# KoryakovDmitry/cuda-mpi-openmp

Hardware: AMD Instinct MI355X
Metric: Gpixel/s lab2 2D conv 4096x4096 + GPU/CPU speedup, at 1/2/4/8 MI355X (higher is better)
Workload: dtype fp32

## Files before the change

### native/src/kernels/edge_kernels.hpp

```cpp
#pragma once

#include <type_traits>

#include "internal.hpp"
#include "peer_sync.hpp"

namespace mpx {
namespace edge {

struct Taps {
    float wx[MPX_MAX_K * MPX_MAX_K];
    float wy[MPX_MAX_K * MPX_MAX_K];
};

struct RowSrc {
    const uint32_t *up = nullptr;
    const uint32_t *dn = nullptr;
    int own_rows = 0x7fffffff;
};

constexpr float kSqrtMargin = 1.0f / 16384.0f;

template <bool FAST>
__device__ __forceinline__ uint32_t mag_to_gray(float s) {
    if constexpr (!FAST) {
        return mpx_sat_u8(sqrtf(s));
    } else {
        if (s >= 65025.0f) return 255u;
        const float r = __builtin_amdgcn_sqrtf(s);
        const float n = truncf(r);
        const float fr = r - n;
        if (fr > kSqrtMargin && fr < 1.0f - kSqrtMargin) return (uint32_t)n;
        return mpx_sat_u8(sqrtf(s));
    }
}

__device__ __forceinline__ void mag2_to_gray(float s0, float s1, uint32_t &g0, uint32_t &g1) {
    const float c0 = __builtin_amdgcn_fmed3f(s0, 0.25f, 65280.25f);
    const float c1 = __builtin_amdgcn_fmed3f(s1, 0.25f, 65280.25f);
    const float r0 = __builtin_amdgcn_sqrtf(c0), r1 = __builtin_amdgcn_sqrtf(c1);
    const float f0 = __builtin_amdgcn_fractf(r0), f1 = __builtin_amdgcn_fractf(r1);
    constexpr float kHalfOpen = 0.5f - kSqrtMargin;
    const bool ok = (int)(fabsf(f0 - 0.5f) < kHalfOpen) & (int)(fabsf(f1 - 0.5f) < kHalfOpen);
    g0 = (uint32_t)r0;
    g1 = (uint32_t)r1;
    if (!ok) {
        g0 = mpx_sat_u8(sqrtf(s0));
        g1 = mpx_sat_u8(sqrtf(s1));
    }
}

typedef float f2_t __attribute__((ext_vector_type(2)));

__device__ __forceinline__ void mag4_to_gray(f2_t s01, f2_t s23, uint32_t g[4]) {
    constexpr float kTwo23 = 8388608.0f;
    const f2_t c01 = {__builtin_amdgcn_fmed3f(s01.x, 0.25f, 65280.25f), __builtin_amdgcn_fmed3f(s01.y, 0.25f, 65280.25f)};
    const f2_t c23 = {__builtin_amdgcn_fmed3f(s23.x, 0.25f, 65280.25f), __builtin_amdgcn_fmed3f(s23.y, 0.25f, 65280.25f)};
    const f2_t r01 = {__builtin_amdgcn_sqrtf(c01.x), __builtin_amdgcn_sqrtf(c01.y)};
    const f2_t r23 = {__builtin_amdgcn_sqrtf(c23.x), __builtin_amdgcn_sqrtf(c23.y)};
    const f2_t kp = {-0.5f + kSqrtMargin, -0.5f + kSqrtMargin}, km = {-0.5f - kSqrtMargin, -0.5f - kSqrtMargin};
    const f2_t big = {kTwo23, kTwo23};
    const f2_t p01 = (r01 + kp) + big, m01 = (r01 + km) + big;
    const f2_t p23 = (r23 + kp) + big, m23 = (r23 + km) + big;
    const bool ok = (int)(p01.x == m01.x) & (int)(p01.y == m01.y) & (int)(p23.x == m23.x) & (int)(p23.y == m23.y);
    if (ok) {
        typedef uint32_t u2_t __attribute__((ext_vector_type(2)));
        const u2_t b01 = __builtin_bit_cast(u2_t, p01), b23 = __builtin_bit_cast(u2_t, p23);
        g[0] = b01.x;
        g[1] = b01.y;
        g[2] = b23.x;
        g[3] = b23.y;
    } else {
        g[0] = mpx_sat_u8(sqrtf(s01.x));
        g[1] = mpx_sat_u8(sqrtf(s01.y));
        g[2] = mpx_sat_u8(sqrtf(s23.x));
        g[3] = mpx_sat_u8(sqrtf(s23.y));
    }
}

template <int MODE, bool FAST>
__device__ __forceinline__ uint32_t finish_gray(float gx, float gy) {
    if constexpr (MODE == MPX_CONV_MAG2) {
        const float a = gx * gx;
        const float b = gy * gy;
        return mag_to_gray<FAST>(a + b);
    } else if constexpr (MODE == MPX_CONV_ABS1) {
        return mpx_sat_u8(fabsf(gx));
    } else {
        return mpx_sat_u8(gx);
    }
}

constexpr int kTX = 64;
constexpr int kTY = 4;
constexpr int kCPT = 2;
constexpr int kTW = kTX * kCPT;
constexpr int kHL = 4;
constexpr int kLW = kTW + 2 * kHL;
constexpr int kNVROW = kLW / 4;

template <bool VEC>
__device__ __forceinline__ uint4 fetch4(const uint32_t *__restrict__ row, int gx, int w) {
    if constexpr (VEC) {
        const int gxc = mpx_clampi(gx, 0, w - 4);
        const uint4 q = *reinterpret_cast<const uint4 *>(row + gxc);
        const bool left = gx < 0, right = gx >= w;
        uint4 p;
        p.x = right ? q.w : q.x;
        p.y = left ? q.x : (right ? q.w : q.y);
        p.z = left ? q.x : (right ? q.w : q.z);
        p.w = left ? q.x : q.w;
        return p;
    } else {
        uint4 p;
        p.x = row[mpx_clampi(gx + 0, 0, w - 1)];
        p.y = row[mpx_clampi(gx + 1, 0, w - 1)];
        p.z = row[mpx_clampi(gx + 2, 0, w - 1)];
        p.w = row[mpx_clampi(gx + 3, 0, w - 1)];
        return p;
    }
}

__device__ __forceinline__ float4 luma4(uint4 p) {
    return make_float4(mpx_luma(p.x), mpx_luma(p.y), mpx_luma(p.z), mpx_luma(p.w));
}

__device__ __forceinline__ uint32_t alpha4(uint4 p) {
    return (p.x >> 24) | ((p.y >> 24) << 8) | ((p.z >> 24) << 16) | (p.w & 0xff000000u);
}

template <int K, int A, int MODE, int RPT, bool FAST>
__device__ __forceinline__ void tile_compute(const float *__restrict__ lum, const Taps &taps, int tx, int ty,
                                             uint32_t (&res)[RPT][kCPT]) {
    constexpr int OFF = (kHL - A) & 1;
    constexpr int NW = (OFF + kCPT + K - 1 + 1) / 2;
    constexpr bool TWO = (MODE == MPX_CONV_MAG2);
    const int wbase = kCPT * tx + kHL - A - OFF;
    float ax[RPT][kCPT], ay[RPT][kCPT];
#pragma unroll
    for (int o = 0; o < RPT; ++o)
#pragma unroll
        for (int j = 0; j < kCPT; ++j) {
            ax[o][j] = 0.0f;
            ay[o][j] = 0.0f;
        }
#pragma unroll
    for (int r = 0; r < RPT + K - 1; ++r) {
        const float *lrow = lum + (ty * RPT + r) * kLW + wbase;
        float wnd[2 * NW];
#pragma unroll
        for (int q = 0; q < NW; ++q) {
            const float2 t = *reinterpret_cast<const float2 *>(lrow + 2 * q);
            wnd[2 * q] = t.x;
            wnd[2 * q + 1] = t.y;
        }
#pragma unroll
        for (int o = 0; o < RPT; ++o) {
            const int dy = r - o;
            if (dy < 0 || dy >= K) continue;
#pragma unroll
            for (int dx = 0; dx < K; ++dx) {
                const float cx = taps.wx[dy * K + dx];
#pragma unroll
                for (int j = 0; j < kCPT; ++j) ax[o][j] = fmaf(cx, wnd[OFF + j + dx], ax[o][j]);
                if constexpr (TWO) {
                    const float cy = taps.wy[dy * K + dx];
#pragma unroll
                    for (int j = 0; j < kCPT; ++j) ay[o][j] = fmaf(cy, wnd[OFF + j + dx], ay[o][j]);
                }
            }
        }
    }
#pragma unroll
    for (int o = 0; o < RPT; ++o)
#pragma unroll
        for (int j = 0; j < kCPT; ++j) res[o][j] = finish_gray<MODE, FAST>(ax[o][j], ay[o][j]);
}

template <int K, int A, int MODE, int RPT, bool VEC, bool FAST>
__global__ __launch_bounds__(256) void conv_stream_kernel(const uint32_t *__restrict__ in, uint32_t *__restrict__ out,
                                                          int w, int pitch, int oy0, int oy1, int y_lo, int y_hi,
                                                          int tiles_y, int chunk, int chunks_per_strip, Taps taps) {
    constexpr int TH = kTY * RPT;
    constexpr int LH = TH + K - 1;
    constexpr int HALO = K - 1;
    constexpr int NEWV = TH * kNVROW;
    constexpr int ITN = (NEWV + 255) / 256;
    constexpr int LUMF = LH * kLW;
    static_assert(A <= kHL && (K - 1 - A) <= kHL, "window exceeds loaded halo");
    static_assert(TH >= HALO, "tile shorter than the window");
    __shared__ __attribute__((aligned(16))) float smem[LUMF + LH * kTW / 4];
    float *lum = smem;
    uint8_t *alpha = reinterpret_cast<uint8_t *>(smem + LUMF);

    const int tid = threadIdx.x;
    const int tx = tid & (kTX - 1);
    const int ty = __builtin_amdgcn_readfirstlane(tid >> 6);
    const int b = xcd_remap(blockIdx.x, gridDim.x);
    const int strip = b / chunks_per_strip;
    const int t0 = (b - strip * chunks_per_strip) * chunk;
    const int t1 = min(t0 + chunk, tiles_y);
    if (t0 >= t1) return;
    const int x0 = strip * kTW;
    const bool full_x = (x0 + kTW <= w);

    auto fetch_rows = [&](uint4 (&regs)[ITN], int gy_first, int nrows_total) {
// ... 319 lines not shown
            r = *reinterpret_cast<const uint2 *>(row + cc);
        } else if constexpr (VEC) {
            const __amdgpu_buffer_rsrc_t rrow = __builtin_amdgcn_make_buffer_rsrc(const_cast<uint32_t *>(row), 0,
                                                                                  w * 4, 0x00020000);
            typedef uint32_t u32x2_t __attribute__((ext_vector_type(2)));
            const u32x2_t v = __builtin_amdgcn_raw_buffer_load_b64(rrow, i <= i_last ? cc * 4 : 0x7ffffff0, 0, 0);
            r = make_uint2(v.x, v.y);
        } else {
            r = make_uint2(row[mpx_clampi(cin, 0, w - 1)], row[mpx_clampi(cin + 1, 0, w - 1)]);
        }
        __builtin_amdgcn_sched_barrier(0);
        return r;
    };
    auto fix_pair = [&](uint2 q) -> uint2 {
        if constexpr (VEC) {
            uint2 p;
            p.x = pair_right ? q.y : q.x;
            p.y = pair_left ? q.x : q.y;
            return p;
        } else {
            return q;
        }
    };

    constexpr int D = K * ((PF + K - 1) / K);
    uint2 pre[D];
    f2_t we[K][NE];
    f2_t wo[K][NO > 0 ? NO : 1];
    f2_t hxr[K], hyr[K];
    uint32_t alp0[K], alp1[K];

    auto consume = [&](int u, uint2 px) {
        const f2_t l = luma2(px.x, px.y);
        alp0[u] = px.x;
        alp1[u] = px.y;
        float wv[NV];
        wv[A] = l.x;
        wv[A + 1] = l.y;
        if constexpr (A >= 1) wv[A - 1] = from_prev(l.y);
        if constexpr (A >= 2) wv[A - 2] = from_prev(l.x);
        if constexpr (A >= 3) wv[A - 3] = from_prev(wv[A - 1]);
        if constexpr (G::R >= 1) wv[A + 2] = from_next(l.x);
        if constexpr (G::R >= 2) wv[A + 3] = from_next(l.y);
        if constexpr (G::R >= 3) wv[A + 4] = from_next(wv[A + 2]);
        if constexpr (SEP) {
            auto pair = [&](int dx) { return f2_t{wv[dx], wv[dx + 1]}; };
            hxr[u] = sep_chain<F, K, 0>(taps, pair);
            if constexpr (TWO) hyr[u] = sep_chain<F, K, 2>(taps, pair);
        } else {
#pragma unroll
            for (int q = 0; q < NE; ++q) we[u][q] = f2_t{wv[2 * q], 2 * q + 1 < NV ? wv[2 * q + 1] : 0.0f};
#pragma unroll
            for (int q = 0; q < NO; ++q) wo[u][q] = f2_t{wv[2 * q + 1], wv[2 * q + 2]};
        }
    };

#pragma unroll
    for (int q = 0; q < D; ++q) pre[q] = load_row(q);
#pragma unroll
    for (int u = 0; u < K - 1; ++u) {
        const uint2 px = fix_pair(pre[u]);
        pre[u] = load_row(u + D);
        consume(u, px);
    }
    auto row_step = [&](auto upc, int g, int v) {
        constexpr bool UP = decltype(upc)::value;
        const int u = (K - 1 + v) % K;
        const int q = (K - 1 + v) % D;
        const int i = K - 1 + g * D + v;
        const uint2 px = fix_pair(pre[q]);
        pre[q] = load_row(i + D);
        consume(u, px);
        const int y = UP ? ye - 1 - (g * D + v) : ys + g * D + v;
        auto slot = [&](int dy) { return UP ? (u + K - dy) % K : (u + 1 + dy) % K; };
        f2_t gx = {0.0f, 0.0f}, gy = {0.0f, 0.0f};
        if constexpr (SEP) {
            gx = sep_chain<F, K, 1>(taps, [&](int dy) { return hxr[slot(dy)]; });
            const float sx = sep_scale<F, K, false>(taps);
            gx = gx * f2_t{sx, sx};
            if constexpr (TWO) {
                gy = sep_chain<F, K, 3>(taps, [&](int dy) { return hyr[slot(dy)]; });
                const float sy = sep_scale<F, K, true>(taps);
                gy = gy * f2_t{sy, sy};
            }
        } else {
            bool sx = false, sy = false;
#pragma unroll
            for (int dy = 0; dy < K; ++dy) {
                const int r = slot(dy);
#pragma unroll
                for (int dx = 0; dx < K; ++dx) {
                    const f2_t pv = (dx & 1) ? wo[r][dx >> 1] : we[r][dx >> 1];
                    tap_step<F::kConst>(gx, sx, tap_x<F>(taps, dy * K + dx), pv);
                    if constexpr (TWO) tap_step<F::kConst>(gy, sy, tap_y<F>(taps, dy * K + dx), pv);
                }
            }
        }
        uint32_t g0, g1;
        if constexpr (TWO) {
            const f2_t sq = gx * gx + gy * gy;
            if constexpr (FAST) {
                mag2_to_gray(sq.x, sq.y, g0, g1);
            } else {
                g0 = mag_to_gray<false>(sq.x);
                g1 = mag_to_gray<false>(sq.y);
            }
        } else {
            g0 = finish_gray<MODE, FAST>(gx.x, 0.0f);
            g1 = finish_gray<MODE, FAST>(gx.y, 0.0f);
        }
        const uint32_t v0 = __builtin_amdgcn_perm(alp0[slot(A)], g0, 0x07000000u);
        const uint32_t v1 = __builtin_amdgcn_perm(alp1[slot(A)], g1, 0x07000000u);
        const bool row_ok = UP ? y >= ys : y < ye;
        const int yc = row_ok ? y : ys;
        const __amdgpu_buffer_rsrc_t orow =
            __builtin_amdgcn_make_buffer_rsrc(out + (int64_t)yc * pitch, 0, row_ok ? w * 4 : 0, 0x00020000);
        constexpr int kDrop = 0x7ffffff0;
        if constexpr (VEC) {
            typedef uint32_t u32x2_t __attribute__((ext_vector_type(2)));
            const u32x2_t pv = {v0, v1};
            __builtin_amdgcn_raw_buffer_store_b64(pv, orow, st0 ? ox * 4 : kDrop, 0, BUFLD == 3 ? 2 : 0);
        } else {
            __builtin_amdgcn_raw_buffer_store_b32(v0, orow, st0 ? ox * 4 : kDrop, 0, 0);
            __builtin_amdgcn_raw_buffer_store_b32(v1, orow, st1 ? ox * 4 + 4 : kDrop, 0, 0);
        }
    };
    const int nrows = ye - ys;
    const int nfull = nrows / D;
    const int rem = nrows - nfull * D;
    auto run = [&](auto upc) {
        for (int g = 0; g < nfull; ++g) {
#pragma unroll
            for (int v = 0; v < D; ++v) row_step(upc, g, v);
        }
        if (rem > 0) {
#pragma unroll
            for (int v = 0; v < D; ++v) {
                if (v >= rem) break;
                row_step(upc, nfull, v);
            }
        }
    };
    if (up) run(std::true_type{});
    else run(std::false_type{});
}

constexpr int kVsRowWords = 64 * 4 + 4;
constexpr int kVsSlotWords = 2 * kVsRowWords;
struct VsX {
    int take_start = -1, give_start = -1, take_end = -1, give_end = -1;
    int ftake_start = 0, fgive_start = 0, ftake_end = 0, fgive_end = 0;
};

template <int K, int A, int MODE, bool FAST, class F, bool UP, int OPT, bool SPW = false, int VSEG = 0>
__device__ __forceinline__ void band4_walk(const uint32_t *__restrict__ in, uint32_t *__restrict__ out,
                                                     int w, int pitch, int ys, int ye, int y_lo, int y_hi, int x0,
                                                     const Taps &taps, RowSrc rs, uint32_t *mbf = nullptr,
                                                     uint32_t *mbl = nullptr, int nf = 0, int nl = 0,
                                                     uint32_t *lds = nullptr, VsX vx = VsX{}) {
    constexpr int R = K - 1 - A;
    constexpr int NV = 4 + A + R;
    constexpr bool TWO = (MODE == MPX_CONV_MAG2);
    constexpr bool SEP = F::kSep;
    typedef uint32_t u32x4_t __attribute__((ext_vector_type(4)));
    typedef uint32_t u32x2_t __attribute__((ext_vector_type(2)));
    const int lane = threadIdx.x & 63;
    constexpr bool up = UP;
    constexpr bool HL = (OPT & 512) != 0;
    const int cin = HL ? x0 - 4 + 4 * lane : x0 + 4 * lane;
    const bool st = HL ? (lane >= 1 && lane <= 62 && cin < w) : cin < w;
    const int cc = HL ? min(max(cin, 0), w - 4) : min(cin, w - 4);
    const bool q_right = cin >= w;
    const bool q_left = HL && cin < 0;
    const bool ap_left = lane == 0, ap_right = lane == 63;
    const bool ap_have = !HL && !(OPT & 16) && ((ap_left && x0 > 0) || (ap_right && x0 + 256 < w));
    constexpr int kDrop = 0x7ffffff0;
    constexpr bool kDppApron = (OPT & (8 | 16 | 512)) == 0;
    constexpr bool BPA = kDppApron && (OPT & 2048) != 0 && !SPW;
    const bool fix_l = kDppApron && ap_left && x0 == 0, fix_r = kDppApron && ap_right && x0 + 256 >= w;
    const int ap_off = ap_have ? (ap_left ? x0 - 2 : x0 + 256) * 4 : (fix_l ? 0 : (fix_r ? cc * 4 + 8 : kDrop));
    const uint32_t ap_selx = fix_r ? 0x07060504u : 0x03020100u;
    const uint32_t ap_sely = fix_l ? 0x03020100u : 0x07060504u;
    if constexpr (VSEG > 0) ye = ys + VSEG;
    const int iy0 = ys - A;
    const int iy_last = ye - 1 + R;
    auto row_ptr = [&](int i) {
        const int gy = mpx_clampi(up ? iy_last - i : iy0 + i, y_lo, y_hi);
        const uint32_t *src = gy < 0 ? rs.up : (gy >= rs.own_rows ? rs.dn : in);
        return src + (int64_t)gy * pitch;
    };
    const int i_last = ye - ys + K - 2;
    static_assert(VSEG == 0 || (A == 2 && K == 5 && VSEG >= 8), "vertical sharing: 5-row windows, 2 + 2 halo rows");
    auto load_row = [&](int i, u32x2_t &ap) -> u32x4_t {
        const uint32_t *row = row_ptr(min(i, i_last));
        int nrec = scalar_le_sel(i, i_last, w * 4);
        if constexpr (VSEG > 0)
            nrec = ((i < 2 && vx.take_start >= 0) || (i >= VSEG + 2 && vx.take_end >= 0)) ? 0 : nrec;
        const __amdgpu_buffer_rsrc_t rr =
            __builtin_amdgcn_make_buffer_rsrc(const_cast<uint32_t *>(row), 0, nrec, 0x00020000);
        const int qo = cc * 4, ao = ap_off;
        u32x4_t q;
        if constexpr (SPW) {
            q = __builtin_amdgcn_raw_buffer_load_b128(rr, qo, 0, peer::kCpolSystem);
            ap = __builtin_amdgcn_raw_buffer_load_b64(rr, ao, 0, peer::kCpolSystem);
        } else if constexpr (HL) {
            q = __builtin_amdgcn_raw_buffer_load_b128(rr, qo, 0, 0);
            ap = u32x2_t{0u, 0u};
        } else if constexpr ((OPT & 8) != 0) {
            q = __builtin_amdgcn_raw_buffer_load_b128(rr, qo, 0, (OPT & 64) ? 2 : 0);
        } else if constexpr (BPA) {
            if ((OPT & 32) && i >= K - 1 && i < ye - ys)
                q = __builtin_amdgcn_raw_buffer_load_b128(rr, qo, 0, 2);
            else
                q = __builtin_amdgcn_raw_buffer_load_b128(rr, qo, 0, 0);
            ap = u32x2_t{0u, 0u};
        } else if ((OPT & 64) || ((OPT & 32) && i >= K - 1 && i < ye - ys)) {
            q = __builtin_amdgcn_raw_buffer_load_b128(rr, qo, 0, 2);
            ap = __builtin_amdgcn_raw_buffer_load_b64(rr, ao, 0, (OPT & 128) ? 0 : 2);
        } else {
            q = __builtin_amdgcn_raw_buffer_load_b128(rr, qo, 0, 0);
            ap = __builtin_amdgcn_raw_buffer_load_b64(rr, ao, 0, 0);
        }
        __builtin_amdgcn_sched_barrier(0);
        return q;
    };
    auto fix_quad = [&](u32x4_t q) -> u32x4_t {
        if constexpr ((OPT & 1024) != 0) return q;
        if constexpr (HL) {
            if (q_left) return u32x4_t{q.x, q.x, q.x, q.x};
        }
        return q_right ? u32x4_t{q.w, q.w, q.w, q.w} : q;
    };
    f2_t ab = {0.0f, 0.0f};
    int bp_addr = 0;
    if constexpr (BPA) {
        const int nload = ye - ys + K - 1;
        const int j = lane >> 1;
        const bool side = lane & 1;
        const bool edge = side ? x0 + 256 >= w : x0 == 0;
        const int col = side ? (edge ? w - 2 : x0 + 256) : (edge ? 0 : x0 - 2);
        const u32x2_t v = *reinterpret_cast<const u32x2_t *>(row_ptr(min(j, nload - 1)) + col);
        ab = luma2((edge && side) ? v.y : v.x, (edge && !side) ? v.x : v.y);
        bp_addr = ap_right ? 4 : 0;
    }
    if constexpr ((OPT & 8) != 0) {
        const int nload = ye - ys + K - 1;
        const int j = lane >> 1, side = lane & 1;
        const bool have = !(OPT & 16) && (side ? x0 + 256 < w : x0 > 0);
        const uint32_t *row = row_ptr(min(j, nload - 1));
        const u32x2_t v = *reinterpret_cast<const u32x2_t *>(row + (have ? (side ? x0 + 256 : x0 - 2) : 0));
        ab = luma2(v.x, v.y);
    }

    constexpr int D = K * ((4 + K - 1) / K);
    u32x4_t pre[D];
    u32x2_t apr[D];
    f2_t hxr[SEP ? K : 1][2], hyr[SEP ? K : 1][2];
    float win[SEP ? 1 : K][NV];
    uint32_t alp[K], alq[K];

    auto consume = [&](int u, u32x4_t px, u32x2_t ap, int ri) {
        const f2_t l01 = luma2(px.x, px.y), l23 = luma2(px.z, px.w);
        alp[u] = __builtin_amdgcn_perm(px.y, px.x, 0x0c0c0703u);
        alq[u] = __builtin_amdgcn_perm(px.w, px.z, 0x0c0c0703u);
        f2_t la;
        if constexpr ((OPT & 8) != 0) {
            auto rl = [&](float x, int l) {
                return __int_as_float(__builtin_amdgcn_readlane(__float_as_int(x), l));
            };
            const f2_t lft = {rl(ab.x, 2 * ri), rl(ab.y, 2 * ri)};
            const f2_t rgt = {rl(ab.x, 2 * ri + 1), rl(ab.y, 2 * ri + 1)};
            la = ap_left ? lft : rgt;
        } else if constexpr (BPA) {
            const int a = bp_addr + 8 * ri;
            la = f2_t{__int_as_float(__builtin_amdgcn_ds_bpermute(a, __float_as_int(ab.x))),
                      __int_as_float(__builtin_amdgcn_ds_bpermute(a, __float_as_int(ab.y)))};
        } else if constexpr (kDppApron) {
            la = luma2(__builtin_amdgcn_perm(ap.y, ap.x, ap_selx), __builtin_amdgcn_perm(ap.y, ap.x, ap_sely));
        } else {
            la = luma2(ap.x, ap.y);
        }
        float wv[NV];
        wv[A + 0] = l01.x;
        wv[A + 1] = l01.y;
        wv[A + 2] = l23.x;
        wv[A + 3] = l23.y;
        if constexpr (kDppApron) {
            if constexpr (A >= 1) wv[A - 1] = shift_or_old<kDppShr1>(la.y, l23.y);
            if constexpr (A >= 2) wv[A - 2] = shift_or_old<kDppShr1>(la.x, l23.x);
            if constexpr (R >= 1) wv[A + 4] = shift_or_old<kDppShl1>(la.x, l01.x);
            if constexpr (R >= 2) wv[A + 5] = shift_or_old<kDppShl1>(la.y, l01.y);
        } else {
            if constexpr (A >= 1) {
                const float d = from_prev(l23.y);
                wv[A - 1] = ap_left ? (ap_have ? la.y : l01.x) : d;
            }
            if constexpr (A >= 2) {
                const float d = from_prev(l23.x);
                wv[A - 2] = ap_left ? (ap_have ? la.x : l01.x) : d;
            }
            if constexpr (R >= 1) {
                const float d = from_next(l01.x);
                wv[A + 4] = ap_right ? (ap_have ? la.x : l23.y) : d;
            }
            if constexpr (R >= 2) {
                const float d = from_next(l01.y);
                wv[A + 5] = ap_right ? (ap_have ? la.y : l23.y) : d;
            }
        }
        if constexpr (SEP && kDppApron && A == 2 && R == 2) {
            const f2_t e0 = {wv[0], wv[1]}, e3 = {wv[6], wv[7]};
            const f2_t pw[7] = {e0, __builtin_shufflevector(e0, l01, 1, 2), l01, __builtin_shufflevector(l01, l23, 1, 2),
                                l23, __builtin_shufflevector(l23, e3, 1, 2), e3};
#pragma unroll
            for (int e = 0; e < 2; ++e) {
                auto pair = [&](int dx) { return pw[2 * e + dx]; };
                hxr[u][e] = sep_chain<F, K, 0>(taps, pair);
                if constexpr (TWO) hyr[u][e] = sep_chain<F, K, 2>(taps, pair);
            }
        } else if constexpr (SEP) {
#pragma unroll
            for (int e = 0; e < 2; ++e) {
                auto pair = [&](int dx) { return f2_t{wv[2 * e + dx], wv[2 * e + dx + 1]}; };
                hxr[u][e] = sep_chain<F, K, 0>(taps, pair);
                if constexpr (TWO) hyr[u][e] = sep_chain<F, K, 2>(taps, pair);
            }
        } else {
#pragma unroll
            for (int j = 0; j < NV; ++j) win[u][j] = wv[j];
        }
    };

    auto vs_put = [&](int slot, int r, u32x4_t q, u32x2_t ap) {
        *reinterpret_cast<u32x4_t *>(lds + slot + r * kVsRowWords + 4 * lane) = q;
        if (ap_left || ap_right)
            *reinterpret_cast<u32x2_t *>(lds + slot + r * kVsRowWords + 256 + (ap_right ? 2 : 0)) = ap;
    };
    auto vs_get = [&](int slot, int r, u32x2_t &ap) -> u32x4_t {
        if (ap_left || ap_right)
            ap = *reinterpret_cast<const u32x2_t *>(lds + slot + r * kVsRowWords + 256 + (ap_right ? 2 : 0));
        return *reinterpret_cast<const u32x4_t *>(lds + slot + r * kVsRowWords + 4 * lane);
    };
    auto vs_flag = [&](int f) { __hip_atomic_store(lds + f, 1u, __ATOMIC_RELEASE, __HIP_MEMORY_SCOPE_WORKGROUP); };
    auto vs_wait = [&](int f) {
        while (__hip_atomic_load(lds + f, __ATOMIC_ACQUIRE, __HIP_MEMORY_SCOPE_WORKGROUP) == 0u)
            __builtin_amdgcn_s_sleep(1);
    };

#pragma unroll
    for (int q = 0; q < D; ++q) pre[q] = load_row(q, apr[q]);
    if constexpr (VSEG > 0) {
        if (vx.give_start >= 0) {
            vs_put(vx.give_start, UP ? 1 : 0, pre[2], apr[2]);
            vs_put(vx.give_start, UP ? 0 : 1, pre[3], apr[3]);
            vs_flag(vx.fgive_start);
        }
        if (vx.take_start >= 0) {
            vs_wait(vx.ftake_start);
            pre[0] = vs_get(vx.take_start, UP ? 1 : 0, apr[0]);
            pre[1] = vs_get(vx.take_start, UP ? 0 : 1, apr[1]);
        }
    }
#pragma unroll
    for (int u = 0; u < K - 1; ++u) {
        const u32x4_t px = fix_quad(pre[u]);
        const u32x2_t ap = apr[u];
        pre[u] = load_row(u + D, apr[u]);
        consume(u, px, ap, u);
    }
    auto row_step = [&](int g, int v) {
        const int u = (K - 1 + v) % K;
        const int q = (K - 1 + v) % D;
        const int i = K - 1 + g * D + v;
        if constexpr (VSEG > 0) {
            if (vx.give_end >= 0 && (i == VSEG || i == VSEG + 1)) {
                vs_put(vx.give_end, UP ? (i == VSEG ? 1 : 0) : (i == VSEG ? 0 : 1), pre[q], apr[q]);
                if (i == VSEG + 1) vs_flag(vx.fgive_end);
            }
            if (vx.take_end >= 0 && (i == VSEG + 2 || i == VSEG + 3)) {
                if (i == VSEG + 2) vs_wait(vx.ftake_end);
                pre[q] = vs_get(vx.take_end, UP ? (i == VSEG + 2 ? 1 : 0) : (i == VSEG + 2 ? 0 : 1), apr[q]);
            }
        }
        const u32x4_t px = fix_quad(pre[q]);
        const u32x2_t ap = apr[q];
        pre[q] = load_row(i + D, apr[q]);
        consume(u, px, ap, i);
        const int y = UP ? ye - 1 - (g * D + v) : ys + g * D + v;
        auto slot = [&](int dy) { return UP ? (u + K - dy) % K : (u + 1 + dy) % K; };
        uint32_t gray[4];
        f2_t sq2[2];
#pragma unroll
        for (int e = 0; e < 2; ++e) {
            f2_t gx = {0.0f, 0.0f}, gy = {0.0f, 0.0f};
            if constexpr (SEP) {
                gx = sep_chain<F, K, 1>(taps, [&](int dy) { return hxr[slot(dy)][e]; });
                const float sx = sep_scale<F, K, false>(taps);
                gx = gx * f2_t{sx, sx};
                if constexpr (TWO) {
                    gy = sep_chain<F, K, 3>(taps, [&](int dy) { return hyr[slot(dy)][e]; });
                    const float sy = sep_scale<F, K, true>(taps);
                    gy = gy * f2_t{sy, sy};
                }
            } else {
                bool sx = false, sy = false;
#pragma unroll
                for (int dy = 0; dy < K; ++dy) {
                    const int r = slot(dy);
#pragma unroll
                    for (int dx = 0; dx < K; ++dx) {
                        const f2_t pv = {win[r][2 * e + dx], win[r][2 * e + dx + 1]};
                        tap_step<F::kConst>(gx, sx, tap_x<F>(taps, dy * K + dx), pv);
                        if constexpr (TWO) tap_step<F::kConst>(gy, sy, tap_y<F>(taps, dy * K + dx), pv);
                    }
                }
            }
            if constexpr (TWO) {
                const f2_t sq = gx * gx + gy * gy;
                if constexpr (FAST) {
                    sq2[e] = sq;
                } else {
                    gray[2 * e] = mag_to_gray<false>(sq.x);
                    gray[2 * e + 1] = mag_to_gray<false>(sq.y);
                }
            } else {
                gray[2 * e] = finish_gray<MODE, FAST>(gx.x, 0.0f);
                gray[2 * e + 1] = finish_gray<MODE, FAST>(gx.y, 0.0f);
            }
        }
        if constexpr (TWO && FAST) mag4_to_gray(sq2[0], sq2[1], gray);
        const uint32_t a = alp[slot(A)], b = alq[slot(A)];
        u32x4_t o;
        o.x = __builtin_amdgcn_perm(a, gray[0], 0x04000000u);
        o.y = __builtin_amdgcn_perm(a, gray[1], 0x05000000u);
        o.z = __builtin_amdgcn_perm(b, gray[2], 0x04000000u);
        o.w = __builtin_amdgcn_perm(b, gray[3], 0x05000000u);
        const bool row_ok = UP ? y >= ys : y < ye;
        const int yc = row_ok ? y : ys;
        const __amdgpu_buffer_rsrc_t orow = __builtin_amdgcn_make_buffer_rsrc(
            out + (int64_t)yc * pitch, 0, UP ? scalar_le_sel(ys, y, w * 4) : scalar_le_sel(y, ye - 1, w * 4), 0x00020000);
        __builtin_amdgcn_raw_buffer_store_b128(o, orow, st ? cin * 4 : kDrop, 0, (OPT & 2) ? 2 : 0);
        if constexpr (SPW) {
            const int own = rs.own_rows;
            const bool mf = mbf != nullptr && y < nf, ml = mbl != nullptr && y >= own - nl;
            uint32_t *mrow = mf ? mbf + (int64_t)y * w : (ml ? mbl + (int64_t)(y - (own - nl)) * w : out);
            const __amdgpu_buffer_rsrc_t mr =
                __builtin_amdgcn_make_buffer_rsrc(mrow, 0, (row_ok && (mf || ml)) ? w * 4 : 0, 0x00020000);
            __builtin_amdgcn_raw_buffer_store_b128(o, mr, st ? cin * 4 : kDrop, 0, peer::kCpolSystem);
        }
    };
    if constexpr (VSEG > 0) {
#pragma unroll
        for (int j = 0; j < VSEG; ++j) row_step(j / D, j % D);
        return;
    }
    const int nrows = ye - ys;
    const int nfull = nrows / D;
    const int rem = nrows - nfull * D;
    for (int g = 0; g < nfull; ++g) {
#pragma unroll
        for (int v = 0; v < D; ++v) row_step(g, v);
    }
    if (rem > 0) {
#pragma unroll
        for (int v = 0; v < D; ++v) {
            if (v >= rem) break;
            row_step(nfull, v);
        }
    }
}

template <int K, int A, int MODE, bool FAST, class F, int OPT = 0, bool SP = false>
__global__ __launch_bounds__((OPT & 4) ? 1024 : 256) __attribute__((amdgpu_waves_per_eu((OPT & 1) ? 5 : 1))) void conv_band4_kernel(const uint32_t *__restrict__ in, uint32_t *__restrict__ out,
                                                         int w, int pitch, int oy0, int oy1, int y_lo, int y_hi,
                                                         int seg, int nwaves, int strips, int alt, Taps taps,
                                                         RowSrc rs, mpx_conv_stream_peer sp) {
    static_assert(A <= 2 && K - 1 - A <= 2, "apron covers two columns on each side");
    constexpr int WPB = (OPT & 4) ? 16 : 4;
    const int gw = xcd_remap(blockIdx.x, gridDim.x) * WPB + __builtin_amdgcn_readfirstlane(threadIdx.x >> 6);
    if (gw >= nwaves) return;
    const int strip = gw % strips;
    const int segs = nwaves / strips;
    const int sg0 = gw / strips;
    const int sg = (!(alt & 2) || segs < 3 || sg0 == 0) ? sg0 : (sg0 == 1 ? segs - 1 : sg0 - 1);
    const int ys = oy0 + sg * seg;
    const int ye = min(ys + seg, oy1);
    constexpr int SW = (OPT & 512) ? 248 : 256;
    if constexpr (SP) {
        constexpr int R = K - 1 - A;
        const bool top = sp.up_flag != nullptr && (ys - A < 0 || ys < sp.n_first);
        const bool bot = sp.dn_flag != nullptr && (ye - 1 + R >= rs.own_rows || ye > rs.own_rows - sp.n_last);
        if (top || bot) {
            const uint32_t c = __hip_atomic_load(sp.sync, __ATOMIC_RELAXED, __HIP_MEMORY_SCOPE_AGENT);
            if (top) peer::wait_at_least(sp.up_flag, c, sp.sync + 64, sp.spin_limit);
            if (bot) peer::wait_at_least(sp.dn_flag, c, sp.sync + 64, sp.spin_limit);
            if (sp.up_flag) rs.up = sp.up_src[c & 1u];
            if (sp.dn_flag) rs.dn = sp.dn_src[c & 1u];
            uint32_t *mbf = top ? sp.mb_first[(c + 1) & 1u] : nullptr;
            uint32_t *mbl = bot ? sp.mb_last[(c + 1) & 1u] : nullptr;
            if ((alt & 1) && (sg & 1))
                band4_walk<K, A, MODE, FAST, F, true, OPT, true>(in, out, w, pitch, ys, ye, y_lo, y_hi, strip * SW,
                                                                 taps, rs, mbf, mbl, sp.n_first, sp.n_last);
            else
                band4_walk<K, A, MODE, FAST, F, false, OPT, true>(in, out, w, pitch, ys, ye, y_lo, y_hi, strip * SW,
                                                                  taps, rs, mbf, mbl, sp.n_first, sp.n_last);
            asm volatile("s_waitcnt vmcnt(0)" ::: "memory");
            if ((threadIdx.x & 63) == 0) {
                const uint32_t n = __hip_atomic_fetch_add(sp.sync + 32, 1u, __ATOMIC_ACQ_REL, __HIP_MEMORY_SCOPE_SYSTEM);
                if (n + 1 == (uint32_t)sp.n_edge) {
                    __hip_atomic_store(sp.sync + 32, 0u, __ATOMIC_RELAXED, __HIP_MEMORY_SCOPE_AGENT);
                    peer::publish(sp.sync, c + 1);
                }
            }
            return;
        }
    }
    constexpr int OIN = (OPT & 512) ? OPT : (OPT | 1024);
    const bool inside = !(OPT & 512) && strip * SW + 256 <= w;
    const bool up = (alt & 1) && (sg & 1);
    if (up) {
        if (inside)
            band4_walk<K, A, MODE, FAST, F, true, OIN>(in, out, w, pitch, ys, ye, y_lo, y_hi, strip * SW, taps, rs);
        else
            band4_walk<K, A, MODE, FAST, F, true, OPT>(in, out, w, pitch, ys, ye, y_lo, y_hi, strip * SW, taps, rs);
    } else {
        if (inside)
            band4_walk<K, A, MODE, FAST, F, false, OIN>(in, out, w, pitch, ys, ye, y_lo, y_hi, strip * SW, taps, rs);
        else
            band4_walk<K, A, MODE, FAST, F, false, OPT>(in, out, w, pitch, ys, ye, y_lo, y_hi, strip * SW, taps, rs);
    }
}

template <int K, int A, int MODE, bool FAST, class F, int VSEG>
__global__ __launch_bounds__(1024) void conv_band16v_kernel(const uint32_t *__restrict__ in, uint32_t *__restrict__ out,
                                                            int w, int pitch, int oy0, int oy1, int y_lo, int y_hi,
                                                            int segs, int strips, Taps taps) {
    constexpr int NB = 15;
    __shared__ __attribute__((aligned(16))) uint32_t xlds[2 * NB * kVsSlotWords + 2 * NB];
    constexpr int kFlag0 = 2 * NB * kVsSlotWords;
    const int wv = __builtin_amdgcn_readfirstlane(threadIdx.x >> 6);
    if (threadIdx.x < 2 * NB) xlds[kFlag0 + threadIdx.x] = 0u;
    __syncthreads();
    const int strip = blockIdx.x % strips;
    const int sg = (blockIdx.x / strips) * 16 + wv;
    if (sg >= segs) return;
    const int ys = oy0 + sg * VSEG;
    const int ye = min(ys + VSEG, oy1);
    auto full = [&](int g) { return g >= 0 && g < segs && oy0 + (g + 1) * VSEG <= oy1; };
    const bool me = full(sg);
    const bool top = me && wv > 0 && full(sg - 1);
    const bool bot = me && wv < 15 && full(sg + 1);
    auto slot = [](int b, int s) { return (2 * b + s) * kVsSlotWords; };
    auto flag = [](int b, int s) { return kFlag0 + 2 * b + s; };
    const bool upw = sg & 1;
    VsX vx;
    const bool st_nb = upw ? bot : top, en_nb = upw ? top : bot;
    const int bs = upw ? wv : wv - 1, be = upw ? wv - 1 : wv;
    if (st_nb) {
        vx.take_start = slot(bs, upw ? 1 : 0);
        vx.give_start = slot(bs, upw ? 0 : 1);
        vx.ftake_start = flag(bs, upw ? 1 : 0);
        vx.fgive_start = flag(bs, upw ? 0 : 1);
    }
    if (en_nb) {
        vx.take_end = slot(be, upw ? 0 : 1);
        vx.give_end = slot(be, upw ? 1 : 0);
        vx.ftake_end = flag(be, upw ? 0 : 1);
        vx.fgive_end = flag(be, upw ? 1 : 0);
    }
    constexpr int OPT = 2 | 64;
    RowSrc rs;
    rs.up = in;
    rs.dn = in;
    if (me) {
        if (upw)
            band4_walk<K, A, MODE, FAST, F, true, OPT, false, VSEG>(in, out, w, pitch, ys, ye, y_lo, y_hi, strip * 256,
                                                                    taps, rs, nullptr, nullptr, 0, 0, xlds, vx);
        else
            band4_walk<K, A, MODE, FAST, F, false, OPT, false, VSEG>(in, out, w, pitch, ys, ye, y_lo, y_hi,
                                                                     strip * 256, taps, rs, nullptr, nullptr, 0, 0,
                                                                     xlds, vx);
    } else {
        if (upw)
            band4_walk<K, A, MODE, FAST, F, true, 34>(in, out, w, pitch, ys, ye, y_lo, y_hi, strip * 256, taps, rs);
        else
            band4_walk<K, A, MODE, FAST, F, false, 34>(in, out, w, pitch, ys, ye, y_lo, y_hi, strip * 256, taps, rs);
    }
}

template <int MODE, bool FAST>
__device__ __forceinline__ uint32_t gray_px(float gx, float gy, uint32_t a) {
    return mpx_px_gray(finish_gray<MODE, FAST>(gx, gy), a);
}

}
}
```

Baseline: 747.3.

## Defer exact sqrt rounding fallback to per-group LDS pass and step row pointers

Replaces the in-line branch on uncertain fast-sqrt rounding with a wave-level ballot. Ambiguous rows are spilled to per-wave LDS and recomputed exactly after each row group, so the hot row loop stays branch-free. Interior bands that need no row clamping or peer sourcing now step load and store row pointers incrementally instead of recomputing clamped addresses. The cost is extra LDS allocation per block, which may lower occupancy, plus more template instantiations and code size.

```diff
diff --git a/native/src/kernels/edge_kernels.hpp b/native/src/kernels/edge_kernels.hpp
--- a/native/src/kernels/edge_kernels.hpp
+++ b/native/src/kernels/edge_kernels.hpp
@@ -52,6 +52,31 @@
 
 typedef float f2_t __attribute__((ext_vector_type(2)));
 
+__device__ __forceinline__ uint64_t mag4_fast(f2_t s01, f2_t s23, uint32_t g[4]) {
+    constexpr float kTwo23 = 8388608.0f;
+    const f2_t c01 = {__builtin_amdgcn_fmed3f(s01.x, 0.25f, 65280.25f), __builtin_amdgcn_fmed3f(s01.y, 0.25f, 65280.25f)};
+    const f2_t c23 = {__builtin_amdgcn_fmed3f(s23.x, 0.25f, 65280.25f), __builtin_amdgcn_fmed3f(s23.y, 0.25f, 65280.25f)};
+    const f2_t r01 = {__builtin_amdgcn_sqrtf(c01.x), __builtin_amdgcn_sqrtf(c01.y)};
+    const f2_t r23 = {__builtin_amdgcn_sqrtf(c23.x), __builtin_amdgcn_sqrtf(c23.y)};
+    const f2_t kp = {-0.5f + kSqrtMargin, -0.5f + kSqrtMargin}, km = {-0.5f - kSqrtMargin, -0.5f - kSqrtMargin};
+    const f2_t big = {kTwo23, kTwo23};
+    const f2_t p01 = (r01 + kp) + big, m01 = (r01 + km) + big;
+    const f2_t p23 = (r23 + kp) + big, m23 = (r23 + km) + big;
+    typedef uint32_t u2_t __attribute__((ext_vector_type(2)));
+    const u2_t b01 = __builtin_bit_cast(u2_t, p01), b23 = __builtin_bit_cast(u2_t, p23);
+    g[0] = b01.x;
+    g[1] = b01.y;
+    g[2] = b23.x;
+    g[3] = b23.y;
+    return __builtin_amdgcn_fcmpf(p01.x, m01.x, 14) | __builtin_amdgcn_fcmpf(p01.y, m01.y, 14) |
+           __builtin_amdgcn_fcmpf(p23.x, m23.x, 14) | __builtin_amdgcn_fcmpf(p23.y, m23.y, 14);
+}
+__device__ __forceinline__ void mag4_exact(f2_t s01, f2_t s23, uint32_t g[4]) {
+    g[0] = mpx_sat_u8(sqrtf(s01.x));
+    g[1] = mpx_sat_u8(sqrtf(s01.y));
+    g[2] = mpx_sat_u8(sqrtf(s23.x));
+    g[3] = mpx_sat_u8(sqrtf(s23.y));
+}
 __device__ __forceinline__ void mag4_to_gray(f2_t s01, f2_t s23, uint32_t g[4]) {
     constexpr float kTwo23 = 8388608.0f;
     const f2_t c01 = {__builtin_amdgcn_fmed3f(s01.x, 0.25f, 65280.25f), __builtin_amdgcn_fmed3f(s01.y, 0.25f, 65280.25f)};
@@ -677,7 +702,8 @@
     int ftake_start = 0, fgive_start = 0, ftake_end = 0, fgive_end = 0;
 };
 
-template <int K, int A, int MODE, bool FAST, class F, bool UP, int OPT, bool SPW = false, int VSEG = 0>
+template <int K, int A, int MODE, bool FAST, class F, bool UP, int OPT, bool SPW = false, int VSEG = 0,
+          bool DEFER = false>
 __device__ __forceinline__ void band4_walk(const uint32_t *__restrict__ in, uint32_t *__restrict__ out,
                                                      int w, int pitch, int ys, int ye, int y_lo, int y_hi, int x0,
                                                      const Taps &taps, RowSrc rs, uint32_t *mbf = nullptr,
@@ -709,15 +735,33 @@
     if constexpr (VSEG > 0) ye = ys + VSEG;
     const int iy0 = ys - A;
     const int iy_last = ye - 1 + R;
-    auto row_ptr = [&](int i) {
-        const int gy = mpx_clampi(up ? iy_last - i : iy0 + i, y_lo, y_hi);
+    constexpr bool RSTEP = (OPT & 1024) != 0;
+    static_assert(!RSTEP || (!SPW && VSEG == 0), "stepped rows: plain interior walks");
+    static_assert(!DEFER || (MODE == MPX_CONV_MAG2 && FAST && VSEG == 0), "deferred exact rows: fast magnitudes");
+    auto img_row = [&](int gy0) {
+        const int gy = mpx_clampi(gy0, y_lo, y_hi);
         const uint32_t *src = gy < 0 ? rs.up : (gy >= rs.own_rows ? rs.dn : in);
         return src + (int64_t)gy * pitch;
     };
+    auto row_ptr = [&](int i) {
+        const int gy = up ? iy_last - i : iy0 + i;
+        if constexpr (RSTEP) return in + (int64_t)gy * pitch;
+        else return img_row(gy);
+    };
+    const int64_t rstep = up ? -(int64_t)pitch : (int64_t)pitch;
+    const uint32_t *lrow = in + (int64_t)(up ? iy_last : iy0) * pitch;
+    uint32_t *srow = out + (int64_t)(up ? ye - 1 : ys) * pitch;
     const int i_last = ye - ys + K - 2;
     static_assert(VSEG == 0 || (A == 2 && K == 5 && VSEG >= 8), "vertical sharing: 5-row windows, 2 + 2 halo rows");
+    const uint32_t n_own = (uint32_t)max(ye - ys - (K - 1), 0);
     auto load_row = [&](int i, u32x2_t &ap) -> u32x4_t {
-        const uint32_t *row = row_ptr(min(i, i_last));
+        const uint32_t *row;
+        if constexpr (RSTEP) {
+            row = lrow;
+            lrow += rstep;
+        } else {
+            row = row_ptr(min(i, i_last));
+        }
         int nrec = scalar_le_sel(i, i_last, w * 4);
         if constexpr (VSEG > 0)
             nrec = ((i < 2 && vx.take_start >= 0) || (i >= VSEG + 2 && vx.take_end >= 0)) ? 0 : nrec;
@@ -734,12 +778,12 @@
         } else if constexpr ((OPT & 8) != 0) {
             q = __builtin_amdgcn_raw_buffer_load_b128(rr, qo, 0, (OPT & 64) ? 2 : 0);
         } else if constexpr (BPA) {
-            if ((OPT & 32) && i >= K - 1 && i < ye - ys)
+            if ((OPT & 32) && (uint32_t)(i - (K - 1)) < n_own)
                 q = __builtin_amdgcn_raw_buffer_load_b128(rr, qo, 0, 2);
             else
                 q = __builtin_amdgcn_raw_buffer_load_b128(rr, qo, 0, 0);
             ap = u32x2_t{0u, 0u};
-        } else if ((OPT & 64) || ((OPT & 32) && i >= K - 1 && i < ye - ys)) {
+        } else if ((OPT & 64) || ((OPT & 32) && (uint32_t)(i - (K - 1)) < n_own)) {
             q = __builtin_amdgcn_raw_buffer_load_b128(rr, qo, 0, 2);
             ap = __builtin_amdgcn_raw_buffer_load_b64(rr, ao, 0, (OPT & 128) ? 0 : 2);
         } else {
@@ -893,6 +937,30 @@
         pre[u] = load_row(u + D, apr[u]);
         consume(u, px, ap, u);
     }
+    typedef float f4_t __attribute__((ext_vector_type(4)));
+    uint32_t pend = 0;
+    auto gray_quad = [](uint32_t a, uint32_t b, const uint32_t (&gray)[4]) {
+        u32x4_t o;
+        o.x = __builtin_amdgcn_perm(a, gray[0], 0x04000000u);
+        o.y = __builtin_amdgcn_perm(a, gray[1], 0x05000000u);
+        o.z = __builtin_amdgcn_perm(b, gray[2], 0x04000000u);
+        o.w = __builtin_amdgcn_perm(b, gray[3], 0x05000000u);
+        return o;
+    };
+    auto store_row = [&](int y, bool row_ok, u32x4_t o, int nrec, bool mb_live) {
+        const int yc = row_ok ? y : ys;
+        const __amdgpu_buffer_rsrc_t orow =
+            __builtin_amdgcn_make_buffer_rsrc(out + (int64_t)yc * pitch, 0, nrec, 0x00020000);
+        __builtin_amdgcn_raw_buffer_store_b128(o, orow, st ? cin * 4 : kDrop, 0, (OPT & 2) ? 2 : 0);
+        if constexpr (SPW) {
+            const int own = rs.own_rows;
+            const bool mf = mbf != nullptr && y < nf, ml = mbl != nullptr && y >= own - nl;
+            uint32_t *mrow = mf ? mbf + (int64_t)y * w : (ml ? mbl + (int64_t)(y - (own - nl)) * w : out);
+            const __amdgpu_buffer_rsrc_t mr =
+                __builtin_amdgcn_make_buffer_rsrc(mrow, 0, (mb_live && (mf || ml)) ? w * 4 : 0, 0x00020000);
+            __builtin_amdgcn_raw_buffer_store_b128(o, mr, st ? cin * 4 : kDrop, 0, peer::kCpolSystem);
+        }
+    };
     auto row_step = [&](int g, int v) {
         const int u = (K - 1 + v) % K;
         const int q = (K - 1 + v) % D;
@@ -953,25 +1021,28 @@
                 gray[2 * e + 1] = finish_gray<MODE, FAST>(gx.y, 0.0f);
             }
         }
-        if constexpr (TWO && FAST) mag4_to_gray(sq2[0], sq2[1], gray);
+        const bool row_ok = UP ? y >= ys : y < ye;
+        int nrec = RSTEP ? scalar_le_sel(i, i_last, w * 4)
+                         : (UP ? scalar_le_sel(ys, y, w * 4) : scalar_le_sel(y, ye - 1, w * 4));
+        bool mb_live = row_ok;
+        if constexpr (TWO && FAST && DEFER) {
+            if (__builtin_expect(mag4_fast(sq2[0], sq2[1], gray) != 0, 0)) {
+                *reinterpret_cast<f4_t *>(lds + (v * 64 + lane) * 4) = f4_t{sq2[0].x, sq2[0].y, sq2[1].x, sq2[1].y};
+                pend |= 1u << v;
+                nrec = 0;
+                mb_live = false;
+            }
+        } else if constexpr (TWO && FAST) {
+            mag4_to_gray(sq2[0], sq2[1], gray);
+        }
         const uint32_t a = alp[slot(A)], b = alq[slot(A)];
-        u32x4_t o;
-        o.x = __builtin_amdgcn_perm(a, gray[0], 0x04000000u);
-        o.y = __builtin_amdgcn_perm(a, gray[1], 0x05000000u);
-        o.z = __builtin_amdgcn_perm(b, gray[2], 0x04000000u);
-        o.w = __builtin_amdgcn_perm(b, gray[3], 0x05000000u);
-        const bool row_ok = UP ? y >= ys : y < ye;
-        const int yc = row_ok ? y : ys;
-        const __amdgpu_buffer_rsrc_t orow = __builtin_amdgcn_make_buffer_rsrc(
-            out + (int64_t)yc * pitch, 0, UP ? scalar_le_sel(ys, y, w * 4) : scalar_le_sel(y, ye - 1, w * 4), 0x00020000);
-        __builtin_amdgcn_raw_buffer_store_b128(o, orow, st ? cin * 4 : kDrop, 0, (OPT & 2) ? 2 : 0);
-        if constexpr (SPW) {
-            const int own = rs.own_rows;
-            const bool mf = mbf != nullptr && y < nf, ml = mbl != nullptr && y >= own - nl;
-            uint32_t *mrow = mf ? mbf + (int64_t)y * w : (ml ? mbl + (int64_t)(y - (own - nl)) * w : out);
-            const __amdgpu_buffer_rsrc_t mr =
-                __builtin_amdgcn_make_buffer_rsrc(mrow, 0, (row_ok && (mf || ml)) ? w * 4 : 0, 0x00020000);
-            __builtin_amdgcn_raw_buffer_store_b128(o, mr, st ? cin * 4 : kDrop, 0, peer::kCpolSystem);
+        const u32x4_t o = gray_quad(a, b, gray);
+        if constexpr (RSTEP) {
+            const __amdgpu_buffer_rsrc_t orow = __builtin_amdgcn_make_buffer_rsrc(srow, 0, nrec, 0x00020000);
+            srow += rstep;
+            __builtin_amdgcn_raw_buffer_store_b128(o, orow, st ? cin * 4 : kDrop, 0, (OPT & 2) ? 2 : 0);
+        } else {
+            store_row(y, row_ok, o, nrec, mb_live);
         }
     };
     if constexpr (VSEG > 0) {
@@ -979,18 +1050,45 @@
         for (int j = 0; j < VSEG; ++j) row_step(j / D, j % D);
         return;
     }
+    auto deferred_rows = [&](int g) {
+        do {
+            const int v = __builtin_ctz(pend);
+            pend &= pend - 1;
+            const int y = UP ? ye - 1 - (g * D + v) : ys + g * D + v;
+            const f4_t s = *reinterpret_cast<const f4_t *>(lds + (v * 64 + lane) * 4);
+            uint32_t gray[4];
+            mag4_exact(f2_t{s.x, s.y}, f2_t{s.z, s.w}, gray);
+            const u32x4_t px = *reinterpret_cast<const u32x4_t *>(img_row(y) + cc);
+            const u32x4_t o = gray_quad(__builtin_amdgcn_perm(px.y, px.x, 0x0c0c0703u),
+                                        __builtin_amdgcn_perm(px.w, px.z, 0x0c0c0703u), gray);
+            store_row(y, true, o, w * 4, true);
+        } while (pend != 0);
+        __builtin_amdgcn_s_waitcnt(0x0f70);
+    };
     const int nrows = ye - ys;
     const int nfull = nrows / D;
     const int rem = nrows - nfull * D;
-    for (int g = 0; g < nfull; ++g) {
-#pragma unroll
-        for (int v = 0; v < D; ++v) row_step(g, v);
-    }
-    if (rem > 0) {
-#pragma unroll
-        for (int v = 0; v < D; ++v) {
-            if (v >= rem) break;
-            row_step(nfull, v);
+    if constexpr (DEFER) {
+        const int ngrp = (nrows + D - 1) / D;
+        for (int g = 0; g < ngrp; ++g) {
+#pragma unroll
+            for (int v = 0; v < D; ++v) {
+                if (v > 0 && g * D + v >= nrows) break;
+                row_step(g, v);
+            }
+            if (pend != 0) deferred_rows(g);
+        }
+    } else {
+        for (int g = 0; g < nfull; ++g) {
+#pragma unroll
+            for (int v = 0; v < D; ++v) row_step(g, v);
+        }
+        if (rem > 0) {
+#pragma unroll
+            for (int v = 0; v < D; ++v) {
+                if (v >= rem) break;
+                row_step(nfull, v);
+            }
         }
     }
 }
@@ -1011,6 +1109,13 @@
     const int ys = oy0 + sg * seg;
     const int ye = min(ys + seg, oy1);
     constexpr int SW = (OPT & 512) ? 248 : 256;
+    constexpr bool DF = MODE == MPX_CONV_MAG2 && FAST && (F::kSep || K < 5);
+    constexpr int DROWS = K * ((4 + K - 1) / K);
+    uint32_t *dq = nullptr;
+    if constexpr (DF) {
+        __shared__ __attribute__((aligned(16))) uint32_t dlds[WPB * DROWS * 64 * 4];
+        dq = dlds + __builtin_amdgcn_readfirstlane(threadIdx.x >> 6) * (DROWS * 64 * 4);
+    }
     if constexpr (SP) {
         constexpr int R = K - 1 - A;
         const bool top = sp.up_flag != nullptr && (ys - A < 0 || ys < sp.n_first);
@@ -1024,11 +1129,11 @@
             uint32_t *mbf = top ? sp.mb_first[(c + 1) & 1u] : nullptr;
             uint32_t *mbl = bot ? sp.mb_last[(c + 1) & 1u] : nullptr;
             if ((alt & 1) && (sg & 1))
-                band4_walk<K, A, MODE, FAST, F, true, OPT, true>(in, out, w, pitch, ys, ye, y_lo, y_hi, strip * SW,
-                                                                 taps, rs, mbf, mbl, sp.n_first, sp.n_last);
+                band4_walk<K, A, MODE, FAST, F, true, OPT, true, 0, DF>(in, out, w, pitch, ys, ye, y_lo, y_hi, strip * SW,
+                                                                        taps, rs, mbf, mbl, sp.n_first, sp.n_last, dq);
             else
-                band4_walk<K, A, MODE, FAST, F, false, OPT, true>(in, out, w, pitch, ys, ye, y_lo, y_hi, strip * SW,
-                                                                  taps, rs, mbf, mbl, sp.n_first, sp.n_last);
+                band4_walk<K, A, MODE, FAST, F, false, OPT, true, 0, DF>(in, out, w, pitch, ys, ye, y_lo, y_hi, strip * SW,
+                                                                         taps, rs, mbf, mbl, sp.n_first, sp.n_last, dq);
             asm volatile("s_waitcnt vmcnt(0)" ::: "memory");
             if ((threadIdx.x & 63) == 0) {
                 const uint32_t n = __hip_atomic_fetch_add(sp.sync + 32, 1u, __ATOMIC_ACQ_REL, __HIP_MEMORY_SCOPE_SYSTEM);
@@ -1041,18 +1146,23 @@
         }
     }
     constexpr int OIN = (OPT & 512) ? OPT : (OPT | 1024);
-    const bool inside = !(OPT & 512) && strip * SW + 256 <= w;
+    const bool rows_in = ys - A >= max(y_lo, 0) && ye - 1 + (K - 1 - A) <= min(y_hi, rs.own_rows - 1);
+    const bool inside = !(OPT & 512) && strip * SW + 256 <= w && rows_in;
     const bool up = (alt & 1) && (sg & 1);
     if (up) {
         if (inside)
-            band4_walk<K, A, MODE, FAST, F, true, OIN>(in, out, w, pitch, ys, ye, y_lo, y_hi, strip * SW, taps, rs);
+            band4_walk<K, A, MODE, FAST, F, true, OIN, false, 0, DF>(in, out, w, pitch, ys, ye, y_lo, y_hi, strip * SW, taps, rs,
+                                                                   nullptr, nullptr, 0, 0, dq);
         else
-            band4_walk<K, A, MODE, FAST, F, true, OPT>(in, out, w, pitch, ys, ye, y_lo, y_hi, strip * SW, taps, rs);
+            band4_walk<K, A, MODE, FAST, F, true, OPT, false, 0, DF>(in, out, w, pitch, ys, ye, y_lo, y_hi, strip * SW, taps, rs,
+                                                                   nullptr, nullptr, 0, 0, dq);
     } else {
         if (inside)
-            band4_walk<K, A, MODE, FAST, F, false, OIN>(in, out, w, pitch, ys, ye, y_lo, y_hi, strip * SW, taps, rs);
+            band4_walk<K, A, MODE, FAST, F, false, OIN, false, 0, DF>(in, out, w, pitch, ys, ye, y_lo, y_hi, strip * SW, taps, rs,
+                                                                   nullptr, nullptr, 0, 0, dq);
         else
-            band4_walk<K, A, MODE, FAST, F, false, OPT>(in, out, w, pitch, ys, ye, y_lo, y_hi, strip * SW, taps, rs);
+            band4_walk<K, A, MODE, FAST, F, false, OPT, false, 0, DF>(in, out, w, pitch, ys, ye, y_lo, y_hi, strip * SW, taps, rs,
+                                                                   nullptr, nullptr, 0, 0, dq);
     }
 }
 
```

Measured after the change: 723.8. -3.1%, worse.
